# google/kubeflow

Hardware: AMD Instinct MI355X
Metric: pytorchjob_train_tokens_per_s (higher is better)
Workload: dtype bf16; 1 GPU; model=llama3-8b, global_batch=7, seq_len=4096, parallelism=dp1

## Files before the change

### kubeflow_amd/models/llama.py

```python
from __future__ import annotations

import math
from dataclasses import dataclass

import torch
import torch.nn as nn
import torch.nn.functional as F

from kubeflow_amd import ops
from kubeflow_amd.parallel import sp as spmod
from kubeflow_amd.parallel import tp as tpmod


@dataclass
class LlamaConfig:
    name: str = "llama3-8b"
    vocab_size: int = 128256
    hidden_size: int = 4096
    n_layers: int = 32
    n_heads: int = 32
    n_kv_heads: int = 8
    head_dim: int = 128
    ffn_dim: int = 14336
    rope_theta: float = 500000.0
# ... 48 lines not shown

def llama_tiny_mha(vocab: int = 512) -> LlamaConfig:
    return LlamaConfig(name="llama-tiny-mha", vocab_size=vocab,
                       hidden_size=256, n_layers=2, n_heads=2, n_kv_heads=2,
                       ffn_dim=512, max_seq_len=512)


class RMSNorm(nn.Module):
    def __init__(self, dim: int, eps: float):
        super().__init__()
        self.weight = nn.Parameter(torch.ones(dim))
        self.eps = eps

    def forward(self, x):
        return ops.rms_norm(x, self.weight, self.eps)


class MoEMLP(nn.Module):

    def __init__(self, cfg: LlamaConfig, ep=None):
        super().__init__()
        h, f, E = cfg.hidden_size, cfg.ffn_dim, cfg.n_experts
        self.cfg = cfg
        self.ep = ep if (ep is not None and ep.world > 1) else None
        n = self.ep.world if self.ep else 1
        if E % n:
            raise ValueError(f"EP degree {n} must divide n_experts ({E})")
        self.local_e = E // n
        self.e_lo = (self.ep.rank if self.ep else 0) * self.local_e
        self.gate = nn.Linear(h, E, bias=False)
# ... 83 lines not shown
        self.mlp_norm = RMSNorm(h, cfg.norm_eps)
        if cfg.n_experts > 0:
            self.moe = MoEMLP(cfg, ep=ep)
            self.w13 = self.w2 = None
        else:
            self.moe = None
            self.w13 = nn.Linear(h, 2 * self.ffn, bias=False)
            self.w2 = nn.Linear(self.ffn, h, bias=False)
        if self.tp:
            for lin in (self.wqkv, self.wo, self.w13, self.w2):
                lin.weight._tp_sharded = True

    def forward(self, x, cos, sin, pos_offset: int = 0, kv_cache=None):
        cfg = self.cfg
        B, S, h = x.shape
        nx = self.attn_norm(x)
        if self.tp:
            nx = tpmod.copy_to(nx, self.tp)
        qkv = F.linear(nx, self.wqkv.weight)
        if kv_cache is not None:
            q, k, v = qkv.split([self.hq * cfg.head_dim,
                                 self.hkv * cfg.head_dim,
                                 self.hkv * cfg.head_dim], dim=-1)
            q = q.view(B, S, self.hq, cfg.head_dim)
            k = k.view(B, S, self.hkv, cfg.head_dim)
            v = v.view(B, S, self.hkv, cfg.head_dim)
            q, k = ops.rope(q, k, cos, sin, pos_offset)
            k, v = kv_cache.update(k, v, pos_offset)
            o = ops.flash_attention(q, k, v, causal=(S > 1))
            o = o.reshape(B, S, self.hq * cfg.head_dim)
        elif self.sp is not None:
# ... 19 lines not shown
                                        self.hkv, cfg.head_dim)
        if self.tp:
            attn = tpmod.reduce_from(
                torch.mm(o.view(B * S, -1), self.wo.weight.t()), self.tp)
            x = (x.view(-1, h) + attn).view(B, S, h)
            ny = tpmod.copy_to(self.mlp_norm(x), self.tp)
            y = ops.swiglu(F.linear(ny, self.w13.weight))
            mlp = tpmod.reduce_from(
                torch.mm(y.view(B * S, self.ffn), self.w2.weight.t()),
                self.tp)
            return (x.view(-1, h) + mlp).view(B, S, h)
        x = torch.addmm(x.view(-1, h), o.view(B * S, -1),
                        self.wo.weight.t()).view(B, S, h)
        if self.moe is not None:
            return x + self.moe(self.mlp_norm(x))
        y = ops.swiglu(F.linear(self.mlp_norm(x), self.w13.weight))
        return torch.addmm(x.view(-1, h), y.view(B * S, cfg.ffn_dim),
                           self.w2.weight.t()).view(B, S, h)


class LlamaModel(nn.Module):
    def __init__(self, cfg: LlamaConfig, device=None, dtype=torch.bfloat16,
                 tp=None, sp=None, ep=None, cp=None):
        super().__init__()
        self.cfg = cfg
        self.tp = tp
        self.sp = sp
        self.ep = ep
        factory = dict(device=device, dtype=dtype)
        with torch.device(device if device is not None else "cpu"):
            self.embed = nn.Embedding(cfg.vocab_size, cfg.hidden_size)
# ... 111 lines not shown
```

### kubeflow_amd/ops/__init__.py

```python
from __future__ import annotations

import ctypes
import os
from typing import Optional

import torch

from . import reference
from . import _backend

__all__ = [
    "rms_norm", "layer_norm", "rope", "flash_attention", "attention_decode",
    "flash_attention_rect", "skinny_linear", "kv_store",
    "decode_rope_store", "skinny_linear_q8", "quantize_fp8_rows",
    "dequantize_fp8_rows",
    "cross_entropy", "fused_adamw", "rope_cos_sin", "native_available",
    "masked_attention",
    "swiglu", "fused_qkv_attention",
]

rope_cos_sin = reference.rope_cos_sin


def native_available() -> bool:
    return _backend.try_load() is not None


def _stream() -> ctypes.c_void_p:
    return ctypes.c_void_p(torch.cuda.current_stream().cuda_stream)


def _p(t: Optional[torch.Tensor]) -> ctypes.c_void_p:
    return ctypes.c_void_p(0 if t is None else t.data_ptr())
# ... 54 lines not shown
        dy2 = dy.contiguous().view(rows, cols)
        dx = torch.empty_like(x2)
        dw = torch.empty_like(weight)
        dw_part = torch.zeros(cols, dtype=torch.float32, device=x2.device)
        _backend.check(
            lib.kf_rmsnorm_bwd(_p(dx), _p(dw), _fp(dw_part), _p(dy2), _p(x2),
                               _p(weight), _fp(rstd), rows, cols, _stream()),
            "rmsnorm_bwd")
        return dx.view(ctx.shape), dw, None


def rms_norm(x: torch.Tensor, weight: torch.Tensor, eps: float = 1e-5):
    if _use_native(x):
        return _RMSNormHip.apply(x, weight, eps)
    return reference.rms_norm(x, weight, eps)



class _RopeHip(torch.autograd.Function):

    @staticmethod
    def forward(ctx, q, k, cos, sin, pos_offset, positions):
        lib = _backend.require()
        B, S, Hq, D = q.shape
        Hkv = k.shape[2]
        q = q.clone(memory_format=torch.contiguous_format)
        k = k.clone(memory_format=torch.contiguous_format)
        _backend.check(
            lib.kf_rope(_p(q), _p(k), _fp(cos), _fp(sin),
                        _ip_or_null(positions), B, S, Hq, Hkv, D,
# ... 673 lines not shown
                          _fp(scale), T, V, ctx.ignore_index, _stream()),
            "ce_bwd")
        return dlogits, None, None, None


def cross_entropy(logits: torch.Tensor, targets: torch.Tensor,
                  ignore_index: int = -100):
    if _use_native(logits):
        inplace_ok = not logits.is_leaf and logits.is_contiguous()
        return _CrossEntropyHip.apply(logits, targets, ignore_index,
                                      inplace_ok)
    return reference.softmax_cross_entropy(logits, targets, ignore_index)



def fused_adamw(p16: torch.Tensor, p32: torch.Tensor, grad: torch.Tensor,
                m: torch.Tensor, v: torch.Tensor,
                wd_mask: Optional[torch.Tensor], lr: float, beta1: float,
                beta2: float, eps: float, weight_decay: float, step: int):
    if p16.is_cuda and _backend.native_enabled():
        lib = _backend.require()
        _backend.check(
            lib.kf_adamw(_p(p16), _fp(p32), _p(grad), _fp(m), _fp(v),
                         _fp(wd_mask), p16.numel(), lr, beta1, beta2, eps,
                         weight_decay, step, _stream()), "adamw")
        return
    g32 = grad.float()
    m.mul_(beta1).add_(g32, alpha=1 - beta1)
    v.mul_(beta2).addcmul_(g32, g32, value=1 - beta2)
    bc1 = 1 - beta1 ** step
    bc2 = 1 - beta2 ** step
    denom = (v / bc2).sqrt().add_(eps)
    decay = weight_decay if wd_mask is None else wd_mask * weight_decay
    p32.mul_(1 - lr * decay)
    p32.addcdiv_(m / bc1, denom, value=-lr)
    p16.copy_(p32.to(torch.bfloat16))
```

### kubeflow_amd/ops/_backend.py

```python
from __future__ import annotations

import ctypes
import os
from pathlib import Path

_LIB_PATH = Path(__file__).resolve().parent / "libkfops.so"
_lib = None
_load_error: str | None = None


def native_enabled() -> bool:
    return os.environ.get("KF_NATIVE_KERNELS", "1") != "0"


def try_load():
    global _lib, _load_error
    if _lib is not None:
        return _lib
    if not native_enabled():
        _load_error = "disabled via KF_NATIVE_KERNELS=0"
        return None
    from . import build_ext
    if build_ext.needs_build():
        try:
# ... 27 lines not shown
_FP = ctypes.POINTER(ctypes.c_float)
_PI64 = ctypes.POINTER(ctypes.c_int64)
_PI32 = ctypes.POINTER(ctypes.c_int32)

_DQ8 = [_P] * 5 + [_FP, _FP] + [_I64] * 7 + [_F, _I32]
_DKV8 = [_P] + _DQ8
_ROPE_TAIL = [_FP, _FP, _I64]
_BWD_HEAD = [_P] * 8 + [_FP, _FP] + [_I64] * 4
_ATTN_BWD = _BWD_HEAD + [_I64] * 5 + [_F, _I32]
_ATTN_FWD = [_P, _FP, _P, _P, _P] + [_I64] * 7 + [_F, _I32, _P]

SIGNATURES: dict[str, list] = {
    "kf_rmsnorm_fwd": [_P, _FP, _P, _P, _I64, _I64, _F, _P],
    "kf_rmsnorm_bwd_nparts": [_I64],
    "kf_rmsnorm_bwd": [_P, _P, _FP, _P, _P, _P, _FP, _I64, _I64, _P],
    "kf_layernorm_fwd": [_P, _FP, _FP, _P, _P, _P, _I64, _I64, _F, _P],
    "kf_layernorm_bwd_nparts": [_I64],
    "kf_layernorm_bwd": [_P, _P, _P, _FP, _P, _P, _P, _FP, _FP, _I64, _I64,
                         _P],
    "kf_rope": [_P, _P, _FP, _FP, _PI64] + [_I64] * 8 + [_I32, _P],
    "kf_swiglu_fwd": [_P, _P, _I64, _I64, _P],
    "kf_swiglu_bwd": [_P, _P, _P, _I64, _I64, _P],
    "kf_adamw": [_P, _FP, _P, _FP, _FP, _FP, _I64, _F, _F, _F, _F, _F, _I64,
                 _P],
    "kf_ce_fwd": [_FP, _FP, _P, _PI64, _I64, _I64, _I64, _P],
    "kf_ce_bwd": [_P, _P, _FP, _PI64, _FP, _I64, _I64, _I64, _P],
    "kf_skinny_gemm": [_P, _P, _P, _P, _FP, _F] + [_I64] * 7 + [_P],
    "kf_skinny_gemm_q8": [_P, _P, _P, _FP, _P, _FP, _F] + [_I64] * 7 + [_P],
    "kf_kv_store": [_P] * 6 + [_I64, _I64, _I64, _P],
    "kf_decode_rope_store": [_P, _P, _P, _P, _FP, _FP, _PI32, _P] +
                            [_I64] * 5 + [_P],
    "kf_attn_fwd": _ATTN_FWD,
    "kf_attn_fwd4": _ATTN_FWD,
    "kf_attn_fwd5": _ATTN_FWD,
    "kf_attn_fwd4_rect": [_P, _FP, _P, _P, _P] + [_I64] * 8 + [_F, _I64, _P],
    "kf_attn_fwd4_abl": [_I32] + _ATTN_FWD,
    "kf_tr16_probe": [_P, _P, _I32, _P],
    "kf_attn_bwd": _ATTN_BWD + [_P],
    "kf_attn_bwd_rope": _ATTN_BWD + _ROPE_TAIL + [_P],
    "kf_attn_bwd8_dq": _DQ8 + [_P],
    "kf_attn_bwd8_dq_rope": _DQ8 + _ROPE_TAIL + [_P],
    "kf_attn_bwd8_dkv": _DKV8 + [_P],
    "kf_attn_bwd8_dkv_rope": _DKV8 + _ROPE_TAIL + [_P],
    "kf_attn_bwd8_dkv_fused": _DKV8 + [_P],
    "kf_attn_bwd8_dkv_fused_rope": _DKV8 + _ROPE_TAIL + [_P],
    "kf_attn64_fwd": [_P, _FP, _P, _P, _P] + [_I64] * 6 + [_F, _I32, _I64,
                                                           _P],
    "kf_attn64_bwd": _BWD_HEAD + [_I64, _I64, _F, _I32, _I64, _P],
    "kf_attn_decode": [_P] * 6 + [_PI32, _PI32] + [_I64] * 6 + [_F, _P],
}
_RETURNS_INT64 = ("kf_rmsnorm_bwd_nparts", "kf_layernorm_bwd_nparts")


def _configure(lib: ctypes.CDLL) -> None:
    for name, argtypes in SIGNATURES.items():
        try:
            fn = getattr(lib, name)
        except AttributeError:
            raise RuntimeError(
                f"{_LIB_PATH.name} does not export {name}: the library and "
                "kubeflow_amd/ops/_backend.py disagree") from None
        fn.restype = _I64 if name in _RETURNS_INT64 else _I32
        fn.argtypes = argtypes


def check(err: int, name: str) -> None:
# ... 3 lines not shown
```

### kubeflow_amd/ops/csrc/adamw.hip

```cpp

#include "kf_common.h"

__global__ void kf_adamw_kernel(unsigned short* __restrict__ p16,
                                float* __restrict__ p32,
                                const unsigned short* __restrict__ g,
                                float* __restrict__ m, float* __restrict__ v,
                                const float* __restrict__ wd_mask, int64_t n4,
                                float lr, float b1, float b2, float eps,
                                float wd, float inv_bc1, float inv_bc2) {
  for (int64_t i = blockIdx.x * (int64_t)blockDim.x + threadIdx.x; i < n4;
       i += gridDim.x * (int64_t)blockDim.x) {
    kf_short4 gv = *reinterpret_cast<const kf_short4*>(g + i * 4);
    kf_float4 pv = *reinterpret_cast<const kf_float4*>(p32 + i * 4);
    kf_float4 mv = *reinterpret_cast<const kf_float4*>(m + i * 4);
    kf_float4 vv = *reinterpret_cast<const kf_float4*>(v + i * 4);
    kf_float4 wdv;
    if (wd_mask) wdv = *reinterpret_cast<const kf_float4*>(wd_mask + i * 4);
    kf_short4 out16;
#pragma unroll
    for (int j = 0; j < 4; ++j) {
      float gf = kf_bf16_to_f32((unsigned short)gv[j]);
      float mf = b1 * mv[j] + (1.f - b1) * gf;
      float vf = b2 * vv[j] + (1.f - b2) * gf * gf;
      float decay = wd_mask ? wdv[j] * wd : wd;
// ... 10 lines not shown
}

KF_EXPORT int kf_adamw(void* p16, float* p32, const void* g, float* m,
                       float* v, const float* wd_mask, int64_t n, float lr,
                       float b1, float b2, float eps, float wd, int64_t step,
                       void* stream) {
  if (n % 4) return (int)hipErrorInvalidValue;
  const float inv_bc1 = 1.f / (1.f - powf(b1, (float)step));
  const float inv_bc2 = 1.f / (1.f - powf(b2, (float)step));
  hipLaunchKernelGGL(kf_adamw_kernel, dim3(kf_grid_for(n / 4, 256)), dim3(256),
                     0, (hipStream_t)stream, (unsigned short*)p16, p32,
                     (const unsigned short*)g, m, v, wd_mask, n / 4, lr, b1,
                     b2, eps, wd, inv_bc1, inv_bc2);
  return (int)hipGetLastError();
}
```

### kubeflow_amd/ops/csrc/kf_ops.h

```cpp
#pragma once

#include <cstdint>

#define KF_EXPORT extern "C" __attribute__((visibility("default")))

KF_EXPORT int kf_rmsnorm_fwd(void* y, float* rstd, const void* x,
    const void* w, int64_t rows, int64_t cols, float eps, void* stream);
KF_EXPORT int64_t kf_rmsnorm_bwd_nparts(int64_t rows);
KF_EXPORT int kf_rmsnorm_bwd(void* dx, void* dw, float* dw_acc, const void* dy,
    const void* x, const void* w, const float* rstd, int64_t rows,
    int64_t cols, void* stream);
KF_EXPORT int kf_layernorm_fwd(void* y, float* mu, float* rstd, const void* x,
    const void* w, const void* b, int64_t rows, int64_t cols, float eps,
    void* stream);
KF_EXPORT int64_t kf_layernorm_bwd_nparts(int64_t rows);
KF_EXPORT int kf_layernorm_bwd(void* dx, void* dw, void* db, float* part,
    const void* dy, const void* x, const void* w, const float* mu,
    const float* rstd, int64_t rows, int64_t cols, void* stream);

KF_EXPORT int kf_rope(void* q, void* k, const float* cost, const float* sint,
    const int64_t* positions, int64_t B, int64_t S, int64_t Hq, int64_t Hkv,
    int64_t D, int64_t qts, int64_t kts, int64_t pos_offset, int backward,
    void* stream);
KF_EXPORT int kf_swiglu_fwd(void* y, const void* h, int64_t T, int64_t F,
    void* stream);
KF_EXPORT int kf_swiglu_bwd(void* dh, const void* dy, const void* h, int64_t T,
    int64_t F, void* stream);
KF_EXPORT int kf_adamw(void* p16, float* p32, const void* g, float* m,
    float* v, const float* wd_mask, int64_t n, float lr, float b1, float b2,
    float eps, float wd, int64_t step, void* stream);
KF_EXPORT int kf_ce_fwd(float* loss_sum, float* lse, const void* logits,
    const int64_t* targets, int64_t T, int64_t V, int64_t ignore_index,
    void* stream);
KF_EXPORT int kf_ce_bwd(void* dlogits, const void* logits, const float* lse,
    const int64_t* targets, const float* scale, int64_t T, int64_t V,
    int64_t ignore_index, void* stream);

KF_EXPORT int kf_skinny_gemm(void* c, const void* a, const void* w,
    const void* res, const float* rmsg, float rms_eps, int64_t swiglu,
    int64_t M, int64_t N, int64_t K, int64_t lda, int64_t ldw, int64_t ldc,
    void* stream);
KF_EXPORT int kf_skinny_gemm_q8(void* c, const void* a, const void* w8,
    const float* wscale, const void* res, const float* rmsg, float rms_eps,
    int64_t swiglu, int64_t M, int64_t N, int64_t K, int64_t lda, int64_t ldw,
    int64_t ldc, void* stream);
// ... 82 lines not shown
```

### kubeflow_amd/ops/csrc/rmsnorm.hip

```cpp

#include "kf_common.h"

#define RN_BLOCK 256
#define RN_VEC 8

__global__ __launch_bounds__(RN_BLOCK) void kf_rmsnorm_fwd_kernel(
    unsigned short* __restrict__ y, float* __restrict__ rstd_out,
    const unsigned short* __restrict__ x, const unsigned short* __restrict__ w,
    int64_t rows, int cols, float eps) {
  __shared__ float scratch[RN_BLOCK / KF_WAVE];
  const int nvec = cols / RN_VEC;
  for (int64_t row = blockIdx.x; row < rows; row += gridDim.x) {
    const unsigned short* xr = x + row * cols;
    unsigned short* yr = y + row * cols;
    float ss = 0.f;
    for (int i = threadIdx.x; i < nvec; i += RN_BLOCK) {
      kf_short8 xv = *reinterpret_cast<const kf_short8*>(xr + i * RN_VEC);
#pragma unroll
      for (int j = 0; j < RN_VEC; ++j) {
        float f = kf_bf16_to_f32((unsigned short)xv[j]);
        ss += f * f;
      }
    }
    ss = kf_block_reduce(ss, scratch, KfSum{}, 0.f);
// ... 2 lines not shown
    for (int i = threadIdx.x; i < nvec; i += RN_BLOCK) {
      kf_short8 xv = *reinterpret_cast<const kf_short8*>(xr + i * RN_VEC);
      kf_short8 wv = *reinterpret_cast<const kf_short8*>(w + i * RN_VEC);
      kf_short8 ov;
#pragma unroll
      for (int j = 0; j < RN_VEC; ++j) {
        float f = kf_bf16_to_f32((unsigned short)xv[j]) * rstd *
                  kf_bf16_to_f32((unsigned short)wv[j]);
        ov[j] = (short)kf_f32_to_bf16(f);
      }
      *reinterpret_cast<kf_short8*>(yr + i * RN_VEC) = ov;
    }
  }
}

__global__ __launch_bounds__(RN_BLOCK) void kf_rmsnorm_bwd_kernel(
    unsigned short* __restrict__ dx, float* __restrict__ dw_part,
    const unsigned short* __restrict__ dy, const unsigned short* __restrict__ x,
    const unsigned short* __restrict__ w, const float* __restrict__ rstd,
    int64_t rows, int cols) {
  extern __shared__ float lds[];
  float* dw_lds = lds;
  float* scratch = lds + cols;
  const int nvec = cols / RN_VEC;
  for (int i = threadIdx.x; i < cols; i += RN_BLOCK) dw_lds[i] = 0.f;
  __syncthreads();

  for (int64_t row = blockIdx.x; row < rows; row += gridDim.x) {
    const unsigned short* dyr = dy + row * cols;
    const unsigned short* xr = x + row * cols;
    unsigned short* dxr = dx + row * cols;
    const float rs = rstd[row];
    float dot = 0.f;
    for (int i = threadIdx.x; i < nvec; i += RN_BLOCK) {
      kf_short8 dyv = *reinterpret_cast<const kf_short8*>(dyr + i * RN_VEC);
// ... 2 lines not shown
#pragma unroll
      for (int j = 0; j < RN_VEC; ++j) {
        float dyf = kf_bf16_to_f32((unsigned short)dyv[j]);
        float xf = kf_bf16_to_f32((unsigned short)xv[j]);
        float wf = kf_bf16_to_f32((unsigned short)wv[j]);
        dot += dyf * wf * xf;
        dw_lds[i * RN_VEC + j] += dyf * xf * rs;
      }
    }
    dot = kf_block_reduce(dot, scratch, KfSum{}, 0.f);
    const float k = rs * rs * rs * dot / (float)cols;
    for (int i = threadIdx.x; i < nvec; i += RN_BLOCK) {
      kf_short8 dyv = *reinterpret_cast<const kf_short8*>(dyr + i * RN_VEC);
      kf_short8 xv = *reinterpret_cast<const kf_short8*>(xr + i * RN_VEC);
      kf_short8 wv = *reinterpret_cast<const kf_short8*>(w + i * RN_VEC);
      kf_short8 ov;
#pragma unroll
      for (int j = 0; j < RN_VEC; ++j) {
        float dyf = kf_bf16_to_f32((unsigned short)dyv[j]);
        float xf = kf_bf16_to_f32((unsigned short)xv[j]);
        float wf = kf_bf16_to_f32((unsigned short)wv[j]);
        ov[j] = (short)kf_f32_to_bf16(rs * dyf * wf - k * xf);
      }
      *reinterpret_cast<kf_short8*>(dxr + i * RN_VEC) = ov;
    }
    __syncthreads();
  }
  for (int i = threadIdx.x; i < cols; i += RN_BLOCK)
    atomicAdd(&dw_part[i], dw_lds[i]);
}

__global__ void kf_cast_bf16_kernel(unsigned short* __restrict__ dst,
                                    const float* __restrict__ src,
                                    int64_t n) {
  for (int64_t i = blockIdx.x * (int64_t)blockDim.x + threadIdx.x; i < n;
       i += gridDim.x * (int64_t)blockDim.x)
    dst[i] = kf_f32_to_bf16(src[i]);
}

KF_EXPORT int kf_rmsnorm_fwd(void* y, float* rstd, const void* x, const void* w,
                             int64_t rows, int64_t cols, float eps,
                             void* stream) {
// ... 7 lines not shown
}

KF_EXPORT int64_t kf_rmsnorm_bwd_nparts(int64_t rows) {
  (void)rows;
  return 1;
}

KF_EXPORT int kf_rmsnorm_bwd(void* dx, void* dw, float* dw_acc,
                             const void* dy, const void* x, const void* w,
                             const float* rstd, int64_t rows, int64_t cols,
                             void* stream) {
  if (cols % RN_VEC) return (int)hipErrorInvalidValue;
  int grid = (int)(rows < 1024 ? rows : 1024);
  if (grid < 1) grid = 1;
  size_t lds = (cols + RN_BLOCK / KF_WAVE) * sizeof(float);
  hipLaunchKernelGGL(kf_rmsnorm_bwd_kernel, dim3(grid), dim3(RN_BLOCK), lds,
                     (hipStream_t)stream, (unsigned short*)dx, dw_acc,
                     (const unsigned short*)dy, (const unsigned short*)x,
                     (const unsigned short*)w, rstd, rows, (int)cols);
  int err = (int)hipGetLastError();
  if (err) return err;
  hipLaunchKernelGGL(kf_cast_bf16_kernel, dim3(kf_grid_for(cols, 256)),
                     dim3(256), 0, (hipStream_t)stream, (unsigned short*)dw,
                     dw_acc, cols);
  return (int)hipGetLastError();
}
```

### kubeflow_amd/parallel/flat.py

```python
from __future__ import annotations

from typing import List, Tuple

import torch
import torch.nn as nn

ALIGN = 64


def _aligned(n: int) -> int:
    return (n + ALIGN - 1) // ALIGN * ALIGN


class FlatParamSpace:
    def __init__(self, model: nn.Module, dtype: torch.dtype | None = None):
        params: List[Tuple[str, nn.Parameter]] = [
            (n, p) for n, p in model.named_parameters() if p.requires_grad]
        params.reverse()
        if dtype is None:
            dtype = params[0][1].dtype
        self.names = [n for n, _ in params]
        device = params[0][1].device
        total = sum(_aligned(p.numel()) for _, p in params)
        self.numel = total
# ... 13 lines not shown

    def zero_grad(self):
        self.grad.zero_()

    def param_offset_end(self, i: int) -> int:
        off, n = self.slices[i]
        return off + _aligned(n)

    def build_wd_mask(self, decay_dim_ge: int = 2) -> torch.Tensor:
        mask = torch.zeros(self.numel, dtype=torch.float32, device=self.device)
        for (off, n), p in zip(self.slices, self.params):
            if p.dim() >= decay_dim_ge:
                mask[off:off + n].fill_(1.0)
        return mask

    def state_dict_tensors(self):
        return list(zip(self.names, (self.data[o:o + n] for o, n in self.slices)))
```

### kubeflow_amd/runtime/trainer.py

```python
from __future__ import annotations

import math
from dataclasses import dataclass
from typing import Optional

import torch

from kubeflow_amd import ops
from kubeflow_amd.parallel import FlatParamSpace, BucketedDDP


@dataclass
class TrainConfig:
    lr: float = 3e-4
    beta1: float = 0.9
    beta2: float = 0.95
    eps: float = 1e-8
    weight_decay: float = 0.1
    warmup_steps: int = 10
    lr_decay_steps: int = 10000
    min_lr_ratio: float = 0.1
    grad_accum: int = 1
    bucket_mb: Optional[float] = None
    use_wd_mask: bool = True
# ... 17 lines not shown
        import torch.distributed as dist
        self.model = model
        self.cfg = cfg
        self.flat = FlatParamSpace(model)
        self.tp = tp_ctx
        self.pp = pp_ctx
        self.ep = ep_ctx
        self.zero = None
        if ep_ctx is not None:
            self.ddp = _NullDDP()
            self.p32 = self.flat.data.float()
            self.m = torch.zeros_like(self.p32)
            self.v = torch.zeros_like(self.p32)
            self.wd_mask = (self.flat.build_wd_mask() if cfg.use_wd_mask
                            else None)
            self.step_num = 0
            return
        if (zero and dist.is_initialized() and dist.get_world_size() > 1
                and tp_ctx is None and pp_ctx is None):
            from kubeflow_amd.parallel.zero import ZeroShard
            self.zero = ZeroShard(self.flat)
            self.ddp = _NullDDP()
            dist.broadcast(self.flat.data, src=0)
            self.p32 = self.zero.data_shard().float()
            self.m = self.zero.new_state()
            self.v = self.zero.new_state()
            if cfg.use_wd_mask:
                full = self.flat.build_wd_mask()
                self.wd_mask = self.zero.shard_of(full).clone()
                del full
            else:
                self.wd_mask = None
            self.step_num = 0
            return
        if tp_ctx is not None and dp_group is not None \
                and dist.get_world_size(dp_group) > 1:
            self.ddp = BucketedDDP(self.flat, bucket_mb=cfg.bucket_mb,
                                   process_group=dp_group)
        elif tp_ctx is not None or pp_ctx is not None:
            self.ddp = _NullDDP()
        else:
            self.ddp = BucketedDDP(self.flat, bucket_mb=cfg.bucket_mb)
        self.p32 = self.flat.data.float()
        self.m = torch.zeros_like(self.p32)
        self.v = torch.zeros_like(self.p32)
        self.wd_mask = self.flat.build_wd_mask() if cfg.use_wd_mask else None
        self.step_num = 0

    def lr_at(self, step: int) -> float:
        cfg = self.cfg
        if step < cfg.warmup_steps:
            return cfg.lr * (step + 1) / max(1, cfg.warmup_steps)
        t = min(1.0, (step - cfg.warmup_steps) /
                max(1, cfg.lr_decay_steps - cfg.warmup_steps))
        floor = cfg.lr * cfg.min_lr_ratio
        return floor + 0.5 * (cfg.lr - floor) * (1 + math.cos(math.pi * t))

    def step(self, *batch) -> torch.Tensor:
        cfg = self.cfg
        self.flat.zero_grad()
        loss = None
# ... 7 lines not shown
                self.ddp.prepare_step()
            loss = self.model(inputs, targets)
            if cfg.grad_accum > 1:
                (loss / cfg.grad_accum).backward()
            else:
                loss.backward()
        self.ddp.finalize()
        if self.ep is not None:
            self.ep.sync_grads(self.flat)
        if self.zero is not None:
            self._zero_update()
        else:
            self._clip_and_update()
        return loss.detach()

    def _clip_and_update(self):
        cfg = self.cfg
        if cfg.grad_clip > 0:
            comm = next((c for c in (self.tp, self.pp, self.ep)
                         if c is not None), None)
            if comm is not None:
                gnorm = comm.global_grad_norm(self.flat)
            else:
                gnorm = torch.linalg.vector_norm(self.flat.grad,
                                                 dtype=torch.float32)
            scale = (cfg.grad_clip / (gnorm + 1e-6)).clamp(max=1.0)
            self.flat.grad.mul_(scale.to(self.flat.grad.dtype))
            self.last_grad_norm = gnorm
        self.step_num += 1
        lr = self.lr_at(self.step_num - 1)
        ops.fused_adamw(self.flat.data, self.p32, self.flat.grad, self.m,
                        self.v, self.wd_mask, lr, cfg.beta1, cfg.beta2,
                        cfg.eps, cfg.weight_decay, self.step_num)

    def _zero_update(self):
        cfg = self.cfg
        gs = self.zero.reduce_scatter_grads()
        if cfg.grad_clip > 0:
            gnorm = self.zero.global_grad_norm(gs)
            scale = (cfg.grad_clip / (gnorm + 1e-6)).clamp(max=1.0)
            gs.mul_(scale.to(gs.dtype))
            self.last_grad_norm = gnorm
        self.step_num += 1
        lr = self.lr_at(self.step_num - 1)
        ops.fused_adamw(self.zero.data_shard(), self.p32, gs, self.m,
                        self.v, self.wd_mask, lr, cfg.beta1, cfg.beta2,
                        cfg.eps, cfg.weight_decay, self.step_num)
        self.zero.all_gather_params()

    def state_dict(self) -> dict:
        return {
            "step": self.step_num,
            "flat_data": self.flat.data,
            "p32": self.p32,
            "m": self.m,
            "v": self.v,
            "param_names": self.flat.names,
            "rng": torch.get_rng_state(),
            "cuda_rng": (torch.cuda.get_rng_state()
                         if torch.cuda.is_available() else None),
        }

# ... 41 lines not shown
```

Before: 21290 tokens/s.

## Fuse residual gradient into RMSNorm backward and fuse grad clip into AdamW

Adds an RMSNorm variant that also returns its input as the residual, so backward can add the residual gradient inside the norm kernel instead of running a separate elementwise add. Adds a register-resident RMSNorm backward kernel for small column counts. The optimizer tail gets a custom bf16 grad sum-of-squares kernel, and the clip scale is folded into a new AdamW kernel that uses uint8 per-64-element weight-decay groups instead of an fp32 mask. Together these cut memory passes over activations and the flat gradient, at the cost of more kernel variants and extra bf16 rounding of the fused residual add.

```diff
diff --git a/kubeflow_amd/models/llama.py b/kubeflow_amd/models/llama.py
--- a/kubeflow_amd/models/llama.py
+++ b/kubeflow_amd/models/llama.py
@@ -86,6 +86,9 @@
 
     def forward(self, x):
         return ops.rms_norm(x, self.weight, self.eps)
+
+    def forward_residual(self, x):
+        return ops.rms_norm_residual(x, self.weight, self.eps)
 
 
 class MoEMLP(nn.Module):
@@ -199,7 +202,11 @@
     def forward(self, x, cos, sin, pos_offset: int = 0, kv_cache=None):
         cfg = self.cfg
         B, S, h = x.shape
-        nx = self.attn_norm(x)
+        res = self.tp is None and self.moe is None
+        if res:
+            nx, x = self.attn_norm.forward_residual(x)
+        else:
+            nx = self.attn_norm(x)
         if self.tp:
             nx = tpmod.copy_to(nx, self.tp)
         qkv = F.linear(nx, self.wqkv.weight)
@@ -249,7 +256,8 @@
                         self.wo.weight.t()).view(B, S, h)
         if self.moe is not None:
             return x + self.moe(self.mlp_norm(x))
-        y = ops.swiglu(F.linear(self.mlp_norm(x), self.w13.weight))
+        ny, x = self.mlp_norm.forward_residual(x)
+        y = ops.swiglu(F.linear(ny, self.w13.weight))
         return torch.addmm(x.view(-1, h), y.view(B * S, cfg.ffn_dim),
                            self.w2.weight.t()).view(B, S, h)
 
diff --git a/kubeflow_amd/ops/__init__.py b/kubeflow_amd/ops/__init__.py
--- a/kubeflow_amd/ops/__init__.py
+++ b/kubeflow_amd/ops/__init__.py
@@ -17,6 +17,7 @@
     "cross_entropy", "fused_adamw", "rope_cos_sin", "native_available",
     "masked_attention",
     "swiglu", "fused_qkv_attention",
+    "rms_norm_residual", "grad_norm", "step_tail_enabled",
 ]
 
 rope_cos_sin = reference.rope_cos_sin
@@ -101,6 +102,64 @@
     if _use_native(x):
         return _RMSNormHip.apply(x, weight, eps)
     return reference.rms_norm(x, weight, eps)
+
+
+def _norm_res_enabled() -> bool:
+    return os.environ.get("KF_NORM_RES", "1") != "0"
+
+
+class _RMSNormResHip(torch.autograd.Function):
+
+    @staticmethod
+    def forward(ctx, x, weight, eps):
+        lib = _backend.require()
+        shape = x.shape
+        x2 = x.contiguous().view(-1, shape[-1])
+        rows, cols = x2.shape
+        y = torch.empty_like(x2)
+        rstd = torch.empty(rows, dtype=torch.float32, device=x.device)
+        _backend.check(
+            lib.kf_rmsnorm_fwd(_p(y), _fp(rstd), _p(x2), _p(weight), rows,
+                               cols, float(eps), _stream()), "rmsnorm_fwd")
+        ctx.save_for_backward(x2, weight, rstd)
+        ctx.shape = shape
+        ctx.set_materialize_grads(False)
+        return y.view(shape), x
+
+    @staticmethod
+    def backward(ctx, dy, dxr):
+        if dy is None:
+            return dxr, None, None
+        lib = _backend.require()
+        x2, weight, rstd = ctx.saved_tensors
+        rows, cols = x2.shape
+        dy2 = dy.contiguous().view(rows, cols)
+        dx = torch.empty_like(x2)
+        dw = torch.empty_like(weight)
+        dw_part = torch.zeros(cols, dtype=torch.float32, device=x2.device)
+        if (dxr is not None and dxr.is_contiguous()
+                and dxr.dtype == dx.dtype and dxr.data_ptr() % 16 == 0):
+            _backend.check(
+                lib.kf_rmsnorm_bwd_res(_p(dx), _p(dw), _fp(dw_part), _p(dy2),
+                                       _p(x2), _p(weight), _fp(rstd),
+                                       _p(dxr), rows, cols, _stream()),
+                "rmsnorm_bwd_res")
+            return dx.view(ctx.shape), dw, None
+        _backend.check(
+            lib.kf_rmsnorm_bwd(_p(dx), _p(dw), _fp(dw_part), _p(dy2), _p(x2),
+                               _p(weight), _fp(rstd), rows, cols, _stream()),
+            "rmsnorm_bwd")
+        dx = dx.view(ctx.shape)
+        return (dx if dxr is None else dx + dxr), dw, None
+
+
+def rms_norm_residual(x: torch.Tensor, weight: torch.Tensor,
+                      eps: float = 1e-5):
+    if _use_native(x):
+        if _norm_res_enabled():
+            return _RMSNormResHip.apply(x, weight, eps)
+        return _RMSNormHip.apply(x, weight, eps), x
+    return reference.rms_norm(x, weight, eps), x
 
 
 
@@ -804,17 +863,64 @@
 
 
 
+WD_GROUP = 64
+
+
+def step_tail_enabled() -> bool:
+    return os.environ.get("KF_STEP_TAIL", "1") != "0"
+
+
+def grad_norm(grad: torch.Tensor) -> torch.Tensor:
+    if (grad.is_cuda and _backend.native_enabled()
+            and grad.dtype == torch.bfloat16 and grad.is_contiguous()
+            and grad.data_ptr() % 16 == 0):
+        lib = _backend.require()
+        n = grad.numel()
+        out = torch.empty(1, dtype=torch.float32, device=grad.device)
+        parts = torch.empty(int(lib.kf_grad_sumsq_nparts(n)),
+                            dtype=torch.float32, device=grad.device)
+        _backend.check(
+            lib.kf_grad_sumsq(_fp(out), _fp(parts), _p(grad), n, _stream()),
+            "grad_sumsq")
+        return out.view(())
+    return torch.linalg.vector_norm(grad, dtype=torch.float32)
+
+
 def fused_adamw(p16: torch.Tensor, p32: torch.Tensor, grad: torch.Tensor,
                 m: torch.Tensor, v: torch.Tensor,
                 wd_mask: Optional[torch.Tensor], lr: float, beta1: float,
-                beta2: float, eps: float, weight_decay: float, step: int):
+                beta2: float, eps: float, weight_decay: float, step: int,
+                wd_groups: Optional[torch.Tensor] = None,
+                gscale: Optional[torch.Tensor] = None):
+    if wd_mask is not None and wd_groups is not None:
+        raise ValueError("fused_adamw: pass wd_mask or wd_groups, not both")
     if p16.is_cuda and _backend.native_enabled():
         lib = _backend.require()
-        _backend.check(
-            lib.kf_adamw(_p(p16), _fp(p32), _p(grad), _fp(m), _fp(v),
-                         _fp(wd_mask), p16.numel(), lr, beta1, beta2, eps,
-                         weight_decay, step, _stream()), "adamw")
+        if wd_groups is None and gscale is None:
+            _backend.check(
+                lib.kf_adamw(_p(p16), _fp(p32), _p(grad), _fp(m), _fp(v),
+                             _fp(wd_mask), p16.numel(), lr, beta1, beta2, eps,
+                             weight_decay, step, _stream()), "adamw")
+            return
+        n = p16.numel()
+        if wd_groups is not None and (
+                wd_groups.dtype != torch.uint8
+                or wd_groups.numel() * WD_GROUP < n):
+            raise ValueError("fused_adamw: wd_groups must be uint8 with one "
+                             f"entry per {WD_GROUP} elements")
+        if gscale is not None and (gscale.dtype != torch.float32
+                                   or gscale.numel() != 1):
+            raise ValueError("fused_adamw: gscale must be one fp32 element")
+        _backend.check(
+            lib.kf_adamw_clip(_p(p16), _fp(p32), _p(grad), _fp(m), _fp(v),
+                              _fp(wd_mask), _p(wd_groups), _fp(gscale), n,
+                              lr, beta1, beta2, eps, weight_decay, step,
+                              _stream()), "adamw_clip")
         return
+    if gscale is not None:
+        grad.mul_(gscale.reshape(()).to(grad.dtype))
+    if wd_groups is not None:
+        wd_mask = wd_groups.float().repeat_interleave(WD_GROUP)[:p16.numel()]
     g32 = grad.float()
     m.mul_(beta1).add_(g32, alpha=1 - beta1)
     v.mul_(beta2).addcmul_(g32, g32, value=1 - beta2)
diff --git a/kubeflow_amd/ops/_backend.py b/kubeflow_amd/ops/_backend.py
--- a/kubeflow_amd/ops/_backend.py
+++ b/kubeflow_amd/ops/_backend.py
@@ -65,6 +65,7 @@
     "kf_rmsnorm_fwd": [_P, _FP, _P, _P, _I64, _I64, _F, _P],
     "kf_rmsnorm_bwd_nparts": [_I64],
     "kf_rmsnorm_bwd": [_P, _P, _FP, _P, _P, _P, _FP, _I64, _I64, _P],
+    "kf_rmsnorm_bwd_res": [_P, _P, _FP, _P, _P, _P, _FP, _P, _I64, _I64, _P],
     "kf_layernorm_fwd": [_P, _FP, _FP, _P, _P, _P, _I64, _I64, _F, _P],
     "kf_layernorm_bwd_nparts": [_I64],
     "kf_layernorm_bwd": [_P, _P, _P, _FP, _P, _P, _P, _FP, _FP, _I64, _I64,
@@ -74,6 +75,10 @@
     "kf_swiglu_bwd": [_P, _P, _P, _I64, _I64, _P],
     "kf_adamw": [_P, _FP, _P, _FP, _FP, _FP, _I64, _F, _F, _F, _F, _F, _I64,
                  _P],
+    "kf_adamw_clip": [_P, _FP, _P, _FP, _FP, _FP, _P, _FP, _I64, _F, _F, _F,
+                      _F, _F, _I64, _P],
+    "kf_grad_sumsq_nparts": [_I64],
+    "kf_grad_sumsq": [_FP, _FP, _P, _I64, _P],
     "kf_ce_fwd": [_FP, _FP, _P, _PI64, _I64, _I64, _I64, _P],
     "kf_ce_bwd": [_P, _P, _FP, _PI64, _FP, _I64, _I64, _I64, _P],
     "kf_skinny_gemm": [_P, _P, _P, _P, _FP, _F] + [_I64] * 7 + [_P],
@@ -100,7 +105,8 @@
     "kf_attn64_bwd": _BWD_HEAD + [_I64, _I64, _F, _I32, _I64, _P],
     "kf_attn_decode": [_P] * 6 + [_PI32, _PI32] + [_I64] * 6 + [_F, _P],
 }
-_RETURNS_INT64 = ("kf_rmsnorm_bwd_nparts", "kf_layernorm_bwd_nparts")
+_RETURNS_INT64 = ("kf_rmsnorm_bwd_nparts", "kf_layernorm_bwd_nparts",
+                  "kf_grad_sumsq_nparts")
 
 
 def _configure(lib: ctypes.CDLL) -> None:
diff --git a/kubeflow_amd/ops/csrc/adamw.hip b/kubeflow_amd/ops/csrc/adamw.hip
--- a/kubeflow_amd/ops/csrc/adamw.hip
+++ b/kubeflow_amd/ops/csrc/adamw.hip
@@ -48,3 +48,149 @@
                      b2, eps, wd, inv_bc1, inv_bc2);
   return (int)hipGetLastError();
 }
+
+
+#define KF_WD_GROUP 64
+
+template <int MASK>
+__global__ void kf_adamw_clip_kernel(
+    unsigned short* __restrict__ p16, float* __restrict__ p32,
+    unsigned short* __restrict__ g, float* __restrict__ m,
+    float* __restrict__ v, const float* __restrict__ wd_mask,
+    const unsigned char* __restrict__ wd_groups,
+    const float* __restrict__ gscale, int64_t n4, float lr, float b1, float b2,
+    float eps, float wd, float inv_bc1, float inv_bc2) {
+  const float s = gscale ? *gscale : 1.f;
+  const bool clip = s != 1.f;
+  for (int64_t i = blockIdx.x * (int64_t)blockDim.x + threadIdx.x; i < n4;
+       i += gridDim.x * (int64_t)blockDim.x) {
+    kf_short4 gv = *reinterpret_cast<const kf_short4*>(g + i * 4);
+    kf_float4 pv = *reinterpret_cast<const kf_float4*>(p32 + i * 4);
+    kf_float4 mv = *reinterpret_cast<const kf_float4*>(m + i * 4);
+    kf_float4 vv = *reinterpret_cast<const kf_float4*>(v + i * 4);
+    kf_float4 wdv;
+    if (MASK == 1) wdv = *reinterpret_cast<const kf_float4*>(wd_mask + i * 4);
+    if (MASK == 2) {
+      const float gm = (float)wd_groups[i / (KF_WD_GROUP / 4)];
+      wdv = (kf_float4){gm, gm, gm, gm};
+    }
+    if (clip) {
+#pragma unroll
+      for (int j = 0; j < 4; ++j)
+        gv[j] = (short)kf_f32_to_bf16(
+            kf_bf16_to_f32((unsigned short)gv[j]) * s);
+      *reinterpret_cast<kf_short4*>(g + i * 4) = gv;
+    }
+    kf_short4 out16;
+#pragma unroll
+    for (int j = 0; j < 4; ++j) {
+      float gf = kf_bf16_to_f32((unsigned short)gv[j]);
+      float mf = b1 * mv[j] + (1.f - b1) * gf;
+      float vf = b2 * vv[j] + (1.f - b2) * gf * gf;
+      float decay = MASK ? wdv[j] * wd : wd;
+      float pf = pv[j] * (1.f - lr * decay);
+      pf -= lr * (mf * inv_bc1) * __frcp_rn(sqrtf(vf * inv_bc2) + eps);
+      mv[j] = mf; vv[j] = vf; pv[j] = pf;
+      out16[j] = (short)kf_f32_to_bf16(pf);
+    }
+    *reinterpret_cast<kf_float4*>(m + i * 4) = mv;
+    *reinterpret_cast<kf_float4*>(v + i * 4) = vv;
+    *reinterpret_cast<kf_float4*>(p32 + i * 4) = pv;
+    *reinterpret_cast<kf_short4*>(p16 + i * 4) = out16;
+  }
+}
+
+KF_EXPORT int kf_adamw_clip(void* p16, float* p32, void* g, float* m, float* v,
+                            const float* wd_mask, const void* wd_groups,
+                            const float* gscale, int64_t n, float lr, float b1,
+                            float b2, float eps, float wd, int64_t step,
+                            void* stream) {
+  if (n % 4 || (wd_mask && wd_groups)) return (int)hipErrorInvalidValue;
+  const float inv_bc1 = 1.f / (1.f - powf(b1, (float)step));
+  const float inv_bc2 = 1.f / (1.f - powf(b2, (float)step));
+  auto kernel = wd_groups ? kf_adamw_clip_kernel<2>
+                : wd_mask ? kf_adamw_clip_kernel<1>
+                          : kf_adamw_clip_kernel<0>;
+  hipLaunchKernelGGL(kernel, dim3(kf_grid_for(n / 4, 256)), dim3(256), 0,
+                     (hipStream_t)stream, (unsigned short*)p16, p32,
+                     (unsigned short*)g, m, v, wd_mask,
+                     (const unsigned char*)wd_groups, gscale, n / 4, lr, b1,
+                     b2, eps, wd, inv_bc1, inv_bc2);
+  return (int)hipGetLastError();
+}
+
+
+#define SSQ_BLOCK 256
+
+__device__ __forceinline__ float kf_sumsq8(kf_short8 gv) {
+  float q[8];
+#pragma unroll
+  for (int j = 0; j < 8; ++j) {
+    float f = kf_bf16_to_f32((unsigned short)gv[j]);
+    q[j] = f * f;
+  }
+  return ((q[0] + q[1]) + (q[2] + q[3])) + ((q[4] + q[5]) + (q[6] + q[7]));
+}
+
+__global__ __launch_bounds__(SSQ_BLOCK) void kf_grad_sumsq_kernel(
+    float* __restrict__ partials, const unsigned short* __restrict__ g,
+    int64_t n) {
+  __shared__ float scratch[SSQ_BLOCK / KF_WAVE];
+  const int64_t n8 = n / 8;
+  const int64_t stride = gridDim.x * (int64_t)SSQ_BLOCK;
+  int64_t i = blockIdx.x * (int64_t)SSQ_BLOCK + threadIdx.x;
+  float a0 = 0.f, a1 = 0.f, a2 = 0.f, a3 = 0.f;
+  for (; i + 3 * stride < n8; i += 4 * stride) {
+    kf_short8 v0 = *reinterpret_cast<const kf_short8*>(g + i * 8);
+    kf_short8 v1 = *reinterpret_cast<const kf_short8*>(g + (i + stride) * 8);
+    kf_short8 v2 =
+        *reinterpret_cast<const kf_short8*>(g + (i + 2 * stride) * 8);
+    kf_short8 v3 =
+        *reinterpret_cast<const kf_short8*>(g + (i + 3 * stride) * 8);
+    a0 += kf_sumsq8(v0);
+    a1 += kf_sumsq8(v1);
+    a2 += kf_sumsq8(v2);
+    a3 += kf_sumsq8(v3);
+  }
+  for (; i < n8; i += stride)
+    a0 += kf_sumsq8(*reinterpret_cast<const kf_short8*>(g + i * 8));
+  if (blockIdx.x == 0 && n8 * 8 + threadIdx.x < n) {
+    float f = kf_bf16_to_f32(g[n8 * 8 + threadIdx.x]);
+    a1 += f * f;
+  }
+  float acc = kf_block_reduce((a0 + a1) + (a2 + a3), scratch, KfSum{}, 0.f);
+  if (threadIdx.x == 0) partials[blockIdx.x] = acc;
+}
+
+__global__ __launch_bounds__(SSQ_BLOCK) void kf_grad_norm_final_kernel(
+    float* __restrict__ out, const float* __restrict__ partials, int nparts) {
+  __shared__ double red[SSQ_BLOCK];
+  double acc = 0.0;
+  for (int i = threadIdx.x; i < nparts; i += SSQ_BLOCK)
+    acc += (double)partials[i];
+  red[threadIdx.x] = acc;
+  __syncthreads();
+  for (int off = SSQ_BLOCK / 2; off > 0; off >>= 1) {
+    if ((int)threadIdx.x < off) red[threadIdx.x] += red[threadIdx.x + off];
+    __syncthreads();
+  }
+  if (threadIdx.x == 0) out[0] = (float)sqrt(red[0]);
+}
+
+KF_EXPORT int64_t kf_grad_sumsq_nparts(int64_t n) {
+  return kf_grid_for(n / 8, SSQ_BLOCK);
+}
+
+KF_EXPORT int kf_grad_sumsq(float* out, float* partials, const void* g,
+                            int64_t n, void* stream) {
+  if (n < 0 || ((uintptr_t)g & 15)) return (int)hipErrorInvalidValue;
+  const int grid = kf_grid_for(n / 8, SSQ_BLOCK);
+  hipLaunchKernelGGL(kf_grad_sumsq_kernel, dim3(grid), dim3(SSQ_BLOCK), 0,
+                     (hipStream_t)stream, partials,
+                     (const unsigned short*)g, n);
+  int err = (int)hipGetLastError();
+  if (err) return err;
+  hipLaunchKernelGGL(kf_grad_norm_final_kernel, dim3(1), dim3(SSQ_BLOCK), 0,
+                     (hipStream_t)stream, out, (const float*)partials, grid);
+  return (int)hipGetLastError();
+}
diff --git a/kubeflow_amd/ops/csrc/kf_ops.h b/kubeflow_amd/ops/csrc/kf_ops.h
--- a/kubeflow_amd/ops/csrc/kf_ops.h
+++ b/kubeflow_amd/ops/csrc/kf_ops.h
@@ -10,6 +10,9 @@
 KF_EXPORT int kf_rmsnorm_bwd(void* dx, void* dw, float* dw_acc, const void* dy,
     const void* x, const void* w, const float* rstd, int64_t rows,
     int64_t cols, void* stream);
+KF_EXPORT int kf_rmsnorm_bwd_res(void* dx, void* dw, float* dw_acc,
+    const void* dy, const void* x, const void* w, const float* rstd,
+    const void* dres, int64_t rows, int64_t cols, void* stream);
 KF_EXPORT int kf_layernorm_fwd(void* y, float* mu, float* rstd, const void* x,
     const void* w, const void* b, int64_t rows, int64_t cols, float eps,
     void* stream);
@@ -29,6 +32,13 @@
 KF_EXPORT int kf_adamw(void* p16, float* p32, const void* g, float* m,
     float* v, const float* wd_mask, int64_t n, float lr, float b1, float b2,
     float eps, float wd, int64_t step, void* stream);
+KF_EXPORT int kf_adamw_clip(void* p16, float* p32, void* g, float* m,
+    float* v, const float* wd_mask, const void* wd_groups,
+    const float* gscale, int64_t n, float lr, float b1, float b2, float eps,
+    float wd, int64_t step, void* stream);
+KF_EXPORT int64_t kf_grad_sumsq_nparts(int64_t n);
+KF_EXPORT int kf_grad_sumsq(float* out, float* partials, const void* g,
+    int64_t n, void* stream);
 KF_EXPORT int kf_ce_fwd(float* loss_sum, float* lse, const void* logits,
     const int64_t* targets, int64_t T, int64_t V, int64_t ignore_index,
     void* stream);
diff --git a/kubeflow_amd/ops/csrc/rmsnorm.hip b/kubeflow_amd/ops/csrc/rmsnorm.hip
--- a/kubeflow_amd/ops/csrc/rmsnorm.hip
+++ b/kubeflow_amd/ops/csrc/rmsnorm.hip
@@ -1,5 +1,7 @@
 
 #include "kf_common.h"
+
+#include <cstdlib>
 
 #define RN_BLOCK 256
 #define RN_VEC 8
@@ -40,11 +42,12 @@
   }
 }
 
+template <bool RES>
 __global__ __launch_bounds__(RN_BLOCK) void kf_rmsnorm_bwd_kernel(
     unsigned short* __restrict__ dx, float* __restrict__ dw_part,
     const unsigned short* __restrict__ dy, const unsigned short* __restrict__ x,
     const unsigned short* __restrict__ w, const float* __restrict__ rstd,
-    int64_t rows, int cols) {
+    const unsigned short* __restrict__ dres, int64_t rows, int cols) {
   extern __shared__ float lds[];
   float* dw_lds = lds;
   float* scratch = lds + cols;
@@ -77,6 +80,10 @@
       kf_short8 dyv = *reinterpret_cast<const kf_short8*>(dyr + i * RN_VEC);
       kf_short8 xv = *reinterpret_cast<const kf_short8*>(xr + i * RN_VEC);
       kf_short8 wv = *reinterpret_cast<const kf_short8*>(w + i * RN_VEC);
+      kf_short8 rv;
+      if (RES)
+        rv = *reinterpret_cast<const kf_short8*>(dres + row * cols +
+                                                 i * RN_VEC);
       kf_short8 ov;
 #pragma unroll
       for (int j = 0; j < RN_VEC; ++j) {
@@ -84,11 +91,105 @@
         float xf = kf_bf16_to_f32((unsigned short)xv[j]);
         float wf = kf_bf16_to_f32((unsigned short)wv[j]);
         ov[j] = (short)kf_f32_to_bf16(rs * dyf * wf - k * xf);
+        if (RES)
+          ov[j] = (short)kf_f32_to_bf16(
+              kf_bf16_to_f32((unsigned short)ov[j]) +
+              kf_bf16_to_f32((unsigned short)rv[j]));
       }
       *reinterpret_cast<kf_short8*>(dxr + i * RN_VEC) = ov;
     }
     __syncthreads();
   }
+  for (int i = threadIdx.x; i < cols; i += RN_BLOCK)
+    atomicAdd(&dw_part[i], dw_lds[i]);
+}
+
+#define RN_REG_SLOTS 2
+#define RN_REG_COLS (RN_REG_SLOTS * RN_BLOCK * RN_VEC)
+
+template <bool RES>
+__global__ __launch_bounds__(RN_BLOCK) void kf_rmsnorm_bwd_reg_kernel(
+    unsigned short* __restrict__ dx, float* __restrict__ dw_part,
+    const unsigned short* __restrict__ dy, const unsigned short* __restrict__ x,
+    const unsigned short* __restrict__ w, const float* __restrict__ rstd,
+    const unsigned short* __restrict__ dres, int64_t rows, int cols) {
+  extern __shared__ float dw_lds[];
+  __shared__ float scratch[RN_BLOCK / KF_WAVE];
+  const int nvec = cols / RN_VEC;
+  float dwacc[RN_REG_SLOTS][RN_VEC];
+  float wf[RN_REG_SLOTS][RN_VEC];
+#pragma unroll
+  for (int t = 0; t < RN_REG_SLOTS; ++t) {
+    const int i = threadIdx.x + t * RN_BLOCK;
+    kf_short8 wv = {0, 0, 0, 0, 0, 0, 0, 0};
+    if (i < nvec) wv = *reinterpret_cast<const kf_short8*>(w + i * RN_VEC);
+#pragma unroll
+    for (int j = 0; j < RN_VEC; ++j) {
+      wf[t][j] = kf_bf16_to_f32((unsigned short)wv[j]);
+      dwacc[t][j] = 0.f;
+    }
+  }
+
+  for (int64_t row = blockIdx.x; row < rows; row += gridDim.x) {
+    const unsigned short* dyr = dy + row * cols;
+    const unsigned short* xr = x + row * cols;
+    unsigned short* dxr = dx + row * cols;
+    const float rs = rstd[row];
+    kf_short8 dyv[RN_REG_SLOTS], xv[RN_REG_SLOTS], rv[RN_REG_SLOTS];
+#pragma unroll
+    for (int t = 0; t < RN_REG_SLOTS; ++t) {
+      const int i = threadIdx.x + t * RN_BLOCK;
+      if (i < nvec) {
+        dyv[t] = *reinterpret_cast<const kf_short8*>(dyr + i * RN_VEC);
+        xv[t] = *reinterpret_cast<const kf_short8*>(xr + i * RN_VEC);
+        if (RES)
+          rv[t] = *reinterpret_cast<const kf_short8*>(dres + row * cols +
+                                                      i * RN_VEC);
+      }
+    }
+    float dot = 0.f;
+#pragma unroll
+    for (int t = 0; t < RN_REG_SLOTS; ++t) {
+      if ((int)threadIdx.x + t * RN_BLOCK < nvec) {
+#pragma unroll
+        for (int j = 0; j < RN_VEC; ++j) {
+          float dyf = kf_bf16_to_f32((unsigned short)dyv[t][j]);
+          float xf = kf_bf16_to_f32((unsigned short)xv[t][j]);
+          dot += dyf * wf[t][j] * xf;
+          dwacc[t][j] += dyf * xf * rs;
+        }
+      }
+    }
+    dot = kf_block_reduce(dot, scratch, KfSum{}, 0.f);
+    const float k = rs * rs * rs * dot / (float)cols;
+#pragma unroll
+    for (int t = 0; t < RN_REG_SLOTS; ++t) {
+      const int i = threadIdx.x + t * RN_BLOCK;
+      if (i < nvec) {
+        kf_short8 ov;
+#pragma unroll
+        for (int j = 0; j < RN_VEC; ++j) {
+          float dyf = kf_bf16_to_f32((unsigned short)dyv[t][j]);
+          float xf = kf_bf16_to_f32((unsigned short)xv[t][j]);
+          ov[j] = (short)kf_f32_to_bf16(rs * dyf * wf[t][j] - k * xf);
+          if (RES)
+            ov[j] = (short)kf_f32_to_bf16(
+                kf_bf16_to_f32((unsigned short)ov[j]) +
+                kf_bf16_to_f32((unsigned short)rv[t][j]));
+        }
+        *reinterpret_cast<kf_short8*>(dxr + i * RN_VEC) = ov;
+      }
+    }
+  }
+#pragma unroll
+  for (int t = 0; t < RN_REG_SLOTS; ++t) {
+    const int i = threadIdx.x + t * RN_BLOCK;
+    if (i < nvec) {
+#pragma unroll
+      for (int j = 0; j < RN_VEC; ++j) dw_lds[i * RN_VEC + j] = dwacc[t][j];
+    }
+  }
+  __syncthreads();
   for (int i = threadIdx.x; i < cols; i += RN_BLOCK)
     atomicAdd(&dw_part[i], dw_lds[i]);
 }
@@ -126,10 +227,11 @@
   int grid = (int)(rows < 1024 ? rows : 1024);
   if (grid < 1) grid = 1;
   size_t lds = (cols + RN_BLOCK / KF_WAVE) * sizeof(float);
-  hipLaunchKernelGGL(kf_rmsnorm_bwd_kernel, dim3(grid), dim3(RN_BLOCK), lds,
-                     (hipStream_t)stream, (unsigned short*)dx, dw_acc,
+  hipLaunchKernelGGL(kf_rmsnorm_bwd_kernel<false>, dim3(grid), dim3(RN_BLOCK),
+                     lds, (hipStream_t)stream, (unsigned short*)dx, dw_acc,
                      (const unsigned short*)dy, (const unsigned short*)x,
-                     (const unsigned short*)w, rstd, rows, (int)cols);
+                     (const unsigned short*)w, rstd,
+                     (const unsigned short*)nullptr, rows, (int)cols);
   int err = (int)hipGetLastError();
   if (err) return err;
   hipLaunchKernelGGL(kf_cast_bf16_kernel, dim3(kf_grid_for(cols, 256)),
@@ -137,3 +239,38 @@
                      dw_acc, cols);
   return (int)hipGetLastError();
 }
+
+static bool kf_rmsnorm_bwd_regs() {
+  static int cached = -1;
+  if (cached < 0) {
+    const char* e = getenv("KF_RMSNORM_BWD_REGS");
+    cached = (e && e[0] == '0') ? 0 : 1;
+  }
+  return cached == 1;
+}
+
+KF_EXPORT int kf_rmsnorm_bwd_res(void* dx, void* dw, float* dw_acc,
+                                 const void* dy, const void* x, const void* w,
+                                 const float* rstd, const void* dres,
+                                 int64_t rows, int64_t cols, void* stream) {
+  if (cols % RN_VEC) return (int)hipErrorInvalidValue;
+  int grid = (int)(rows < 1024 ? rows : 1024);
+  if (grid < 1) grid = 1;
+  const bool regs = cols <= RN_REG_COLS && kf_rmsnorm_bwd_regs();
+  size_t lds = (cols + (regs ? 0 : RN_BLOCK / KF_WAVE)) * sizeof(float);
+  auto kernel = regs ? (dres ? kf_rmsnorm_bwd_reg_kernel<true>
+                             : kf_rmsnorm_bwd_reg_kernel<false>)
+                     : (dres ? kf_rmsnorm_bwd_kernel<true>
+                             : kf_rmsnorm_bwd_kernel<false>);
+  hipLaunchKernelGGL(kernel, dim3(grid), dim3(RN_BLOCK), lds,
+                     (hipStream_t)stream, (unsigned short*)dx, dw_acc,
+                     (const unsigned short*)dy, (const unsigned short*)x,
+                     (const unsigned short*)w, rstd,
+                     (const unsigned short*)dres, rows, (int)cols);
+  int err = (int)hipGetLastError();
+  if (err) return err;
+  hipLaunchKernelGGL(kf_cast_bf16_kernel, dim3(kf_grid_for(cols, 256)),
+                     dim3(256), 0, (hipStream_t)stream, (unsigned short*)dw,
+                     dw_acc, cols);
+  return (int)hipGetLastError();
+}
diff --git a/kubeflow_amd/parallel/flat.py b/kubeflow_amd/parallel/flat.py
--- a/kubeflow_amd/parallel/flat.py
+++ b/kubeflow_amd/parallel/flat.py
@@ -51,5 +51,13 @@
                 mask[off:off + n].fill_(1.0)
         return mask
 
+    def build_wd_groups(self, decay_dim_ge: int = 2) -> torch.Tensor:
+        groups = torch.zeros(self.numel // ALIGN, dtype=torch.uint8,
+                             device=self.device)
+        for (off, n), p in zip(self.slices, self.params):
+            if p.dim() >= decay_dim_ge:
+                groups[off // ALIGN:(off + _aligned(n)) // ALIGN].fill_(1)
+        return groups
+
     def state_dict_tensors(self):
         return list(zip(self.names, (self.data[o:o + n] for o, n in self.slices)))
diff --git a/kubeflow_amd/runtime/trainer.py b/kubeflow_amd/runtime/trainer.py
--- a/kubeflow_amd/runtime/trainer.py
+++ b/kubeflow_amd/runtime/trainer.py
@@ -55,6 +55,8 @@
             self.v = torch.zeros_like(self.p32)
             self.wd_mask = (self.flat.build_wd_mask() if cfg.use_wd_mask
                             else None)
+            self.wd_groups = (self.flat.build_wd_groups()
+                              if cfg.use_wd_mask else None)
             self.step_num = 0
             return
         if (zero and dist.is_initialized() and dist.get_world_size() > 1
@@ -72,6 +74,12 @@
                 del full
             else:
                 self.wd_mask = None
+            self.wd_groups = None
+            if cfg.use_wd_mask and self.zero.lo % ops.WD_GROUP == 0:
+                g_lo = self.zero.lo // ops.WD_GROUP
+                g_hi = -(-self.zero.hi // ops.WD_GROUP)
+                self.wd_groups = \
+                    self.flat.build_wd_groups()[g_lo:g_hi].clone()
             self.step_num = 0
             return
         if tp_ctx is not None and dp_group is not None \
@@ -86,6 +94,8 @@
         self.m = torch.zeros_like(self.p32)
         self.v = torch.zeros_like(self.p32)
         self.wd_mask = self.flat.build_wd_mask() if cfg.use_wd_mask else None
+        self.wd_groups = (self.flat.build_wd_groups() if cfg.use_wd_mask
+                          else None)
         self.step_num = 0
 
     def lr_at(self, step: int) -> float:
@@ -123,38 +133,54 @@
             self._clip_and_update()
         return loss.detach()
 
+    def _fused_tail(self, grad: torch.Tensor) -> bool:
+        return (ops.step_tail_enabled() and grad.is_cuda
+                and grad.dtype == torch.bfloat16 and ops.native_available())
+
+    def _update(self, p16, grad, scale, fused: bool):
+        cfg = self.cfg
+        gscale = None
+        if scale is not None:
+            if fused:
+                gscale = scale.to(grad.dtype).float().reshape(1)
+            else:
+                grad.mul_(scale.to(grad.dtype))
+        mask, groups = self.wd_mask, None
+        if fused and self.wd_groups is not None:
+            mask, groups = None, self.wd_groups
+        self.step_num += 1
+        lr = self.lr_at(self.step_num - 1)
+        ops.fused_adamw(p16, self.p32, grad, self.m, self.v, mask, lr,
+                        cfg.beta1, cfg.beta2, cfg.eps, cfg.weight_decay,
+                        self.step_num, wd_groups=groups, gscale=gscale)
+
     def _clip_and_update(self):
         cfg = self.cfg
+        grad = self.flat.grad
+        fused = self._fused_tail(grad)
+        scale = None
         if cfg.grad_clip > 0:
             comm = next((c for c in (self.tp, self.pp, self.ep)
                          if c is not None), None)
             if comm is not None:
                 gnorm = comm.global_grad_norm(self.flat)
-            else:
-                gnorm = torch.linalg.vector_norm(self.flat.grad,
-                                                 dtype=torch.float32)
+            elif fused:
+                gnorm = ops.grad_norm(grad)
+            else:
+                gnorm = torch.linalg.vector_norm(grad, dtype=torch.float32)
             scale = (cfg.grad_clip / (gnorm + 1e-6)).clamp(max=1.0)
-            self.flat.grad.mul_(scale.to(self.flat.grad.dtype))
             self.last_grad_norm = gnorm
-        self.step_num += 1
-        lr = self.lr_at(self.step_num - 1)
-        ops.fused_adamw(self.flat.data, self.p32, self.flat.grad, self.m,
-                        self.v, self.wd_mask, lr, cfg.beta1, cfg.beta2,
-                        cfg.eps, cfg.weight_decay, self.step_num)
+        self._update(self.flat.data, grad, scale, fused)
 
     def _zero_update(self):
         cfg = self.cfg
         gs = self.zero.reduce_scatter_grads()
+        scale = None
         if cfg.grad_clip > 0:
             gnorm = self.zero.global_grad_norm(gs)
             scale = (cfg.grad_clip / (gnorm + 1e-6)).clamp(max=1.0)
-            gs.mul_(scale.to(gs.dtype))
             self.last_grad_norm = gnorm
-        self.step_num += 1
-        lr = self.lr_at(self.step_num - 1)
-        ops.fused_adamw(self.zero.data_shard(), self.p32, gs, self.m,
-                        self.v, self.wd_mask, lr, cfg.beta1, cfg.beta2,
-                        cfg.eps, cfg.weight_decay, self.step_num)
+        self._update(self.zero.data_shard(), gs, scale, self._fused_tail(gs))
         self.zero.all_gather_params()
 
     def state_dict(self) -> dict:
```

Result: faster. 21570 tokens/s, median of 6 (+1.3%).
